# bxh1/VIDO-SLAM

Hardware: AMD Instinct MI355X
Metric: frames/sec end-to-end (flow+depth+track+local-BA) at 640x480; BA iters/sec (higher is better)
Workload: dtype f32

## Files before the change

### include/vido_c.h

```cpp
#ifndef VIDO_C_H
#define VIDO_C_H
#include <stdint.h>
#include <stddef.h>
#ifdef __cplusplus
extern "C" {
#endif

#define VIDO_OK              0
#define VIDO_E_INVALID      -1
#define VIDO_E_NO_DEVICE    -2
#define VIDO_E_HIP          -3
#define VIDO_E_CAPACITY     -4
#define VIDO_E_NOMEM        -5

#define VIDO_MAX_LEVELS 16

typedef struct vido_ctx vido_ctx;

typedef struct vido_keypoint { float x, y, size, angle, response; int32_t octave; } vido_keypoint;

typedef struct vido_config {
    int32_t device;
    int32_t width, height;
    int32_t max_batch;
// ... 115 lines not shown

typedef int (*vido_allreduce_fn)(void* user, void* dev_ptr, size_t count, int op);

int vido_ba_optimize(vido_ctx* ctx, vido_ba_problem* prob, vido_ba_result* result, vido_allreduce_fn allreduce, void* user);
int vido_rccl_unique_id(uint8_t id_out[128]);
int vido_rccl_init(vido_ctx* ctx, const uint8_t id[128], int rank, int world);
int vido_rccl_allreduce(void* user_ctx, void* dev_ptr, size_t count, int op);
int vido_rccl_destroy(vido_ctx* ctx);

typedef struct vido_ba_dynamic {
    int32_t n_H, n_dyn, n_tern, n_smooth;
    double* H_T;
    double* dyn_xyz;
    const int32_t* dyn_cam; const double* dyn_meas;
    const int32_t* tern_prev; const int32_t* tern_cur; const int32_t* tern_H;
    const int32_t* sm_i; const int32_t* sm_j;
    double info_dyn, info_tern, info_smooth, huber_dyn, huber_tern, huber_smooth;
} vido_ba_dynamic;
int vido_ba_optimize_dynamic(vido_ctx* ctx, vido_ba_problem* prob, vido_ba_dynamic* dyn, vido_ba_result* result,
                             vido_allreduce_fn allreduce, void* user);

int vido_correlation(vido_ctx* ctx, const float* first, const float* second, int B, int C, int H, int W, int stride,
                     float* out, int on_device);
int vido_det_order(vido_ctx* ctx, const float* scores, const long long* labels, const int* n_det, float confidence, int cap, long long* order, long long* labels_out, long long* n_live);
int vido_roi_levels(vido_ctx* ctx, const float* boxes, int n, float k_min, float k_max, int* out);
int vido_mask_logit_select(vido_ctx* ctx, const float* feat, const float* w, const float* b, const long long* labels, float* out, int n, int c, int hw, int classes);
int vido_bias_act(vido_ctx* ctx, float* x, const float* bias, int N, int C, int H, int W, float slope);
int vido_bias_unary(vido_ctx* ctx, float* x, const float* bias, int N, int C, int H, int W, int kind);
int vido_upcat_reflect(vido_ctx* ctx, const float* x, const float* skip, int C1, int C2, int h, int w, float* out);
int vido_minmax_norm_u16(vido_ctx* ctx, const float* d, const float* mm, int64_t n, int32_t* out);
int vido_bias_res_act(vido_ctx* ctx, float* x, const float* bias, const float* res, int N, int C, int H, int W, float slope);
int vido_area_feed(vido_ctx* ctx, const uint8_t* bgr, int H, int W, float* out, int OH, int OW, float div);
int vido_backwarp(vido_ctx* ctx, const float* x, const float* flow, int B, int C, int H, int W, float* out);
int vido_deconv4s2_depthwise(vido_ctx* ctx, const float* x, const float* weight, int B, int C, int H, int W, float input_slope, float* out);

int vido_conv1x1_supported(int cin, int cout, int hw);
int vido_conv1x1_layout(int cin, int cout, int hw);
int vido_conv1x1_set_arith(int arith);
int vido_conv1x1_range_flag(vido_ctx* ctx, int reset);
int vido_range_latch(vido_ctx* ctx, unsigned* dst);
int vido_conv1x1_bias_act(vido_ctx* ctx, const float* x, const float* w_packed, const float* bias, const float* residual, float* y, int cin, int cout, int hw, float slope);
int vido_deconv2x2_supported(int n, int cin, int cout, int h, int w);
int vido_deconv2x2_bias_act(vido_ctx* ctx, const float* x, const float* w_packed, const float* bias, float* y, int n, int cin, int cout, int h, int w, float slope);
int vido_conv1x1_bias_up2_act(vido_ctx* ctx, const float* x, const float* w_packed, const float* bias, const float* residual_half, float* y, int cin, int cout, int h, int w, float slope);

int vido_conv_kxk_c2(vido_ctx* ctx, const float* x, const float* w, const float* bias, const float* residual, float* y, int cin, int k, int h, int w_);
int vido_conv1x1_skinny(vido_ctx* ctx, const float* x, const float* w_packed, const float* bias, const float* residual, float* y, int cin, int cout, long long hw, float slope);

int vido_conv_direct_supported(int cin, int cout, int h, int w, int kh, int kw, int sh, int sw, int ph, int pw);
long long vido_conv_direct_packed_floats(int cin, int cout, int kh, int kw);
int vido_conv_direct_pack(const float* w, int cin, int cout, int kh, int kw, float* w_packed);
int vido_conv_direct_bias_act(vido_ctx* ctx, const float* x, const float* w_packed, const float* bias, float* y, int n, int cin, int cout, int h, int w,
                              int kh, int kw, int sh, int sw, int ph, int pw, float slope);

int vido_wino3x3_supported(int cin, int cout, int h, int w);
int vido_wino3x3_fills_chip(int n, int cout, int h, int w, int min_wgs);
long long vido_wino3x3_packed_floats(int cin, int cout);
int vido_wino3x3_pack(const float* w, int cin, int cout, float* u_packed);
int vido_wino3x3_bias_act(vido_ctx* ctx, const float* x, const float* u_packed, const float* bias, float* y, int n, int cin, int cout, int h, int w, float slope);
int vido_wino3x3_form(int n, int cin, int cout, int h, int w);
int vido_fc_h_splitk(int rows, int k, int outs);
int vido_fc_h(vido_ctx* ctx, const float* x, const void* w_packed, const float* bias, float* part, float* y, int rows, int k, int outs, float slope);
int vido_conv3x3_h_supported(int n, int cin, int cout, int h, int w);
int vido_conv3x3_h_workgroups(int n, int cout, int h, int w);
int vido_conv3x3_h_bias_act(vido_ctx* ctx, const float* x, const void* w_packed, const float* bias, float* y, int n, int cin, int cout, int h, int w, float slope);
long long vido_wino3x3_packed_floats_form(int cin, int cout, int form);
int vido_wino3x3_pack_form(const float* w, int cin, int cout, int form, float* u_packed);
int vido_wino3x3_bias_act_form(vido_ctx* ctx, const float* x, const float* u_packed, const float* bias, float* y, int n, int cin, int cout, int h, int w, float slope, int form);
int vido_gconv3x3_supported(int H, int W, int cpg_in, int cpg_out);
int64_t vido_gconv3x3_packed_size(int groups, int cpg_in, int cpg_out);
int vido_gconv3x3_bias_act(vido_ctx* ctx, const float* x, const float* in_bias, const float* w_packed, const float* bias, float* y, int groups, int cpg_in, int cpg_out, int H, int W, float slope);
int vido_gconv3x3_s2_supported(int H, int W, int cpg_in, int cpg_out);
int vido_gconv3x3_s2_bias_act(vido_ctx* ctx, const float* x, const float* w_packed, const float* bias, float* y, int groups, int cpg_in, int cpg_out, int H, int W, float slope);
int vido_lfn_reg_front(vido_ctx* ctx, const float* im1, const float* im2, const float* flow, const float* mean, float scale, int B, int C, int H, int W, float* out, int out_channels);
int vido_lfn_reg_tail(vido_ctx* ctx, const float* dist, const float* flow, const float* wx, const float* bx, const float* wy, const float* by, int B, int K, int H, int W, float* out);
int vido_roi_align(vido_ctx* ctx, const float* feat, int B, int C, int H, int W, const float* rois, int n_rois,
                   float spatial_scale, int pooled_h, int pooled_w, int sampling_ratio, float* out, int on_device);
int vido_nms(vido_ctx* ctx, const float* boxes_xyxy, const float* scores, int n, float thresh, int32_t* keep_out,
             int32_t* n_keep, int on_device);
int vido_nms_grouped(vido_ctx* ctx, const float* boxes_xyxy, const float* scores, const int32_t* groups, int n, float thresh,
                     int32_t* keep_out, int32_t* n_keep, int on_device);
int vido_nms_segments(vido_ctx* ctx, const float* boxes_xyxy, const int32_t* groups, const int32_t* seg_off, const int32_t* seg_n, int n_seg, int max_n, int total,
                      float thresh, int32_t* keep_out, int32_t* n_keep);
int vido_roi_align_fpn(vido_ctx* ctx, const float* const feat[4], const int H[4], const int W[4], const float scale[4], int C, const float* boxes, const int32_t* level,
                       int n, int pooled_h, int pooled_w, int sampling_ratio, float* out);
int vido_nchw_to_nhwc(vido_ctx* ctx, const float* src, int B, int C, int H, int W, float* dst);
int vido_roi_align_fpn_nhwc(vido_ctx* ctx, const float* const feat[4], const int H[4], const int W[4], const float scale[4], int C, const float* boxes, const int32_t* level,
                            int n, int pooled_h, int pooled_w, int sampling_ratio, float* out);
int vido_bawin_create(vido_ctx* ctx, int cap_frames, int cap_features);
int vido_bawin_push_frame(vido_ctx* ctx, int frame, int n, const double* meas, const float* xyz, const int32_t* asso);
int vido_bawin_set_labels(vido_ctx* ctx, int n, const int32_t* quads);
int vido_bawin_solve(vido_ctx* ctx, int start, int N, vido_ba_problem* prob, vido_ba_result* res, int32_t* n_obs_out, int32_t* n_pt_out);
int vido_bawin_read_points(vido_ctx* ctx, int frame, int n, float* xyz_out);
int vido_rpn_select(vido_ctx* ctx, int n_levels, const float* const* logits, const float* const* deltas, const int* h, const int* w, const int* stride, const float* cell_anchors,
                    int A, int K, int img_w, int img_h, float* boxes_out, float* scores_out, int32_t* n_out);
int vido_rpn_merge(vido_ctx* ctx, const float* boxes, const float* scores, const int32_t* keep, const int32_t* cnt, int n_levels, int K, int post_nms_top_n, int n_final,
                   float* out_boxes, float* out_scores, int32_t* n_valid);
int vido_det_class_sort(vido_ctx* ctx, const float* prob, const float* deltas, const float* proposals, const float* objectness, int N, int nc, float thresh, const float weights[4],
                        int img_w, int img_h, float* seg_boxes, int32_t* order, int32_t* seg_n);
int vido_det_select(vido_ctx* ctx, const float* prob, const float* seg_boxes, const int32_t* order, const int32_t* keep, const int32_t* cnt, int N, int nc, int detections_per_img, int cap,
                    int32_t* scratch, float* out_boxes, float* out_scores, int64_t* out_labels, int32_t* n_det);
int vido_mask_label_image(vido_ctx* ctx, const float* masks, const float* boxes, const int64_t* labels, int n, int M, int padding, float thresh, int H, int W, uint8_t* out);
int vido_box_decode(vido_ctx* ctx, const float* deltas, const float* boxes, int n, int k, const float weights[4],
                    float* out, int on_device);

int vido_pnp_ransac(vido_ctx* ctx, const float* pts3d, const float* pts2d, int n, double fx, double fy, double cx, double cy,
// ... 60 lines not shown
```

### vido-slam_amd/build.py

```python
import os, subprocess, glob, hashlib

HERE = os.path.dirname(os.path.abspath(__file__))
CSRC = os.path.join(HERE, "csrc")
LIB = os.path.join(HERE, "libvido_slam_hip.so")
import shlex as _shlex
FLAGS = _shlex.split(os.environ.get("VIDO_EXTRA_FLAGS", "")) + ["--offload-arch=gfx950", "-O3", "-std=c++17", "-fPIC", "-shared", "-ffp-contract=off",
         "-fno-fast-math", "-munsafe-fp-atomics", "-Wall", "-Wno-unused-function", "-Wno-unused-result", "-Wno-unused-value", "-pthread"]


def sources():
    return sorted(glob.glob(os.path.join(CSRC, "*.hip")) + glob.glob(os.path.join(CSRC, "*.cpp")))


def _stamp():
    h = hashlib.sha1()
    for p in sources() + sorted(glob.glob(os.path.join(CSRC, "*.hpp"))) + sorted(glob.glob(os.path.join(HERE, "..", "include", "*.h"))):
        h.update(open(p, "rb").read())
    h.update(" ".join(FLAGS).encode())
    return h.hexdigest()


def _obj_stamp(src):
    h = hashlib.sha1()
    h.update(open(src, "rb").read())
    for p in sorted(glob.glob(os.path.join(CSRC, "*.hpp"))) + sorted(glob.glob(os.path.join(HERE, "..", "include", "*.h"))) + sorted(glob.glob(os.path.join(HERE, "..", "include", "vido_slam", "*.h"))):
        h.update(open(p, "rb").read())
    h.update(" ".join(FLAGS + _file_flags(src)).encode())
    return h.hexdigest()


FILE_FLAGS = {"convdirect": ["-mllvm", "-amdgpu-mfma-vgpr-form"]}


_PROBED = {}


def _flag_ok(flags):
    key = " ".join(flags)
    if key not in _PROBED:
        import tempfile
        with tempfile.TemporaryDirectory() as d:
            src = os.path.join(d, "probe.hip"); open(src, "w").write("__global__ void k() {}\n")
            r = subprocess.run([os.environ.get("HIPCC", "/opt/rocm/bin/hipcc"), "--offload-arch=gfx950", "-c", "-x", "hip", src, "-o", os.path.join(d, "probe.o")] + flags,
                               stdout=subprocess.DEVNULL, stderr=subprocess.DEVNULL)
        _PROBED[key] = r.returncode == 0
    return _PROBED[key]


def _file_flags(src):
    stem = os.path.basename(src).split(".")[0]
    ff = FILE_FLAGS.get(stem, [])
    if ff and not _flag_ok(ff):
        ff = []
    return ff + _shlex.split(os.environ.get("VIDO_FLAGS_" + stem, ""))


def build(force=False, verbose=False, lib=None):
    lib = lib or LIB
    stamp_file = lib + ".stamp"
    stamp = _stamp() + "".join(" ".join(_file_flags(x)) for x in sources())
    if not force and os.path.exists(lib) and os.path.exists(stamp_file) and open(stamp_file).read() == stamp:
        return lib
    hipcc = os.environ.get("HIPCC", "/opt/rocm/bin/hipcc")
    objdir = os.path.join(HERE, "build")
    os.makedirs(objdir, exist_ok=True)
    cflags = [f for f in FLAGS if f != "-shared"]
    jobs, objs = [], []
    for s in sources():
        o = os.path.join(objdir, os.path.basename(s) + "." + _obj_stamp(s)[:16] + ".o")
        objs.append(o)
        if force or not os.path.exists(o):
            jobs.append([hipcc] + cflags + _file_flags(s) + ["-c", "-x", "hip", s, "-o", o])
    if jobs:
        from concurrent.futures import ThreadPoolExecutor
        def run(cmd):
            if verbose:
                print(" ".join(cmd))
            subprocess.check_call(cmd)
        with ThreadPoolExecutor(max_workers=min(len(jobs), os.cpu_count() or 4)) as ex:
            list(ex.map(run, jobs))
    subprocess.check_call([hipcc, "--offload-arch=gfx950", "-shared", "-fPIC", "-pthread", "-o", lib] + objs)
    live = set(objs)
    for o in glob.glob(os.path.join(objdir, "*.o")):
        if o not in live and lib == LIB:
# ... 20 lines not shown
```

### vido-slam_amd/nets/fuse.py

```python
import os
import torch
import torch.nn as nn
import torch.nn.functional as F


def _fold(conv, bn, eps):
    scale = bn.weight * (bn.running_var + eps).rsqrt()
    w = conv.weight * scale.reshape(-1, 1, 1, 1)
    b = bn.bias - bn.running_mean * scale
    if conv.bias is not None:
        b = b + conv.bias * scale
    return w.detach().contiguous(), b.detach().contiguous()


def _eps(bn):
    return float(getattr(bn, "eps", 0.0))


def fold_batchnorm(net, ops):
    from .maskrcnn import _Bottleneck, _Stem
    from .monodepth2 import _Basic, ResnetEncoder18, DepthDecoder
    n = 0
    for m in net.modules():
        if isinstance(m, _Bottleneck):
            m._w1, m._b1 = _fold(m.conv1, m.bn1, _eps(m.bn1)); m._w2, m._b2 = _fold(m.conv2, m.bn2, _eps(m.bn2)); m._w3, m._b3 = _fold(m.conv3, m.bn3, _eps(m.bn3)); n += 3
            if m.downsample is not None:
                m._wd, m._bd = _fold(m.downsample[0], m.downsample[1], _eps(m.downsample[1])); n += 1
            m._ep = ops.bias_res_act_
            c2 = m.conv2; m._w2p = None; m._ops = ops
            if c2.groups > 1 and tuple(c2.stride) == (1, 1) and tuple(c2.padding) == (1, 1) and tuple(c2.dilation) == (1, 1) and not os.environ.get("VIDO_NO_GCONV"):
                from .ops import pack_gconv3x3
                m._w2p = pack_gconv3x3(m._w2, c2.groups)
            elif (c2.groups > 1 and tuple(c2.stride) == (2, 2) and tuple(c2.padding) == (1, 1) and tuple(c2.dilation) == (1, 1) and ((c2.out_channels // c2.groups) % 32 == 0 or (c2.out_channels // c2.groups) in (8, 16))
                  and not os.environ.get("VIDO_NO_GCONV") and not os.environ.get("VIDO_NO_GCONV_S2")):
                from .ops import pack_gconv3x3
                m._w2p = pack_gconv3x3(m._w2, c2.groups)
            m._w1p = m._w3p = m._wdp = None; m._c1x1_min_tiles = 0
            mode = os.environ.get("VIDO_CONV1X1", "all")
            if not os.environ.get("VIDO_NO_CONV1X1") and hasattr(ops, "conv1x1_bias_act"):
                from .ops import PackedConv1x1
                m._w3p = PackedConv1x1.make(m._w3)
                if mode == "all":
                    if tuple(m.conv1.stride) == (1, 1): m._w1p = PackedConv1x1.make(m._w1)
                    if m.downsample is not None and tuple(m.downsample[0].stride) in ((1, 1), (2, 2)): m._wdp = PackedConv1x1.make(m._wd)
        elif isinstance(m, _Stem):
            m._w1, m._b1 = _fold(m.conv1, m.bn1, _eps(m.bn1)); m._ep = ops.bias_res_act_; n += 1
        elif isinstance(m, _Basic):
            m._w1, m._b1 = _fold(m.conv1, m.bn1, m.bn1.eps); m._w2, m._b2 = _fold(m.conv2, m.bn2, m.bn2.eps); n += 2
            if m.downsample is not None:
                m._wd, m._bd = _fold(m.downsample[0], m.downsample[1], m.downsample[1].eps); n += 1
            m._ep = ops.bias_res_act_
        elif isinstance(m, DepthDecoder):
            m._ops = ops if hasattr(ops, "upcat_reflect") and not os.environ.get("VIDO_NO_DEPTH_FUSED") else None
        elif isinstance(m, ResnetEncoder18):
            e = m.encoder
            w, b = _fold(e.conv1, e.bn1, e.bn1.eps)
            m._w1, m._b1 = w, b; m._ep = ops.bias_res_act_; n += 1
    return n


class Graphed:

    def __init__(self, fn, example_inputs, warmup=2):
        self.fn = fn
        self.static_in = [x.clone() for x in example_inputs]
        side = torch.cuda.Stream()
        side.wait_stream(torch.cuda.current_stream())
        with torch.cuda.stream(side):
            for _ in range(warmup):
                fn(*self.static_in)
        torch.cuda.current_stream().wait_stream(side)
        torch.cuda.synchronize()
        self.graph = torch.cuda.CUDAGraph()
        with torch.cuda.graph(self.graph):
            self.static_out = fn(*self.static_in)
        torch.cuda.synchronize()

    def __call__(self, *inputs):
        for d, s in zip(self.static_in, inputs):
            if d.data_ptr() != s.data_ptr():
                d.copy_(s, non_blocking=True)
        self.graph.replay()
        return self.static_out
```

### vido-slam_amd/nets/monodepth2.py

```python
import torch
import torch.nn as nn
import torch.nn.functional as F


class _Basic(nn.Module):
    def __init__(self, cin, cout, stride):
        super().__init__()
        self.conv1 = nn.Conv2d(cin, cout, 3, stride, 1, bias=False); self.bn1 = nn.BatchNorm2d(cout)
        self.conv2 = nn.Conv2d(cout, cout, 3, 1, 1, bias=False); self.bn2 = nn.BatchNorm2d(cout)
        self.downsample = None
        if stride != 1 or cin != cout:
            self.downsample = nn.Sequential(nn.Conv2d(cin, cout, 1, stride, bias=False), nn.BatchNorm2d(cout))

    _ep = None

    def forward(self, x):
        if self._ep is not None and x.is_cuda:
            ep = self._ep
            y = ep(F.conv2d(x, self._w1, None, self.conv1.stride, 1), self._b1, None, 0.0)
            sc = x if self.downsample is None else ep(F.conv2d(x, self._wd, None, self.downsample[0].stride), self._bd, None, 1.0)
            return ep(F.conv2d(y, self._w2, None, 1, 1), self._b2, sc.contiguous(), 0.0)
        y = F.relu(self.bn1(self.conv1(x)))
        y = self.bn2(self.conv2(y))
        return F.relu(y + (x if self.downsample is None else self.downsample(x)))


class _ResNet18Trunk(nn.Module):
    def __init__(self):
        super().__init__()
        self.conv1 = nn.Conv2d(3, 64, 7, 2, 3, bias=False); self.bn1 = nn.BatchNorm2d(64)
        self.layer1 = nn.Sequential(_Basic(64, 64, 1), _Basic(64, 64, 1))
        self.layer2 = nn.Sequential(_Basic(64, 128, 2), _Basic(128, 128, 1))
        self.layer3 = nn.Sequential(_Basic(128, 256, 2), _Basic(256, 256, 1))
        self.layer4 = nn.Sequential(_Basic(256, 512, 2), _Basic(512, 512, 1))
        self.fc = nn.Linear(512, 1000)


class ResnetEncoder18(nn.Module):
    num_ch_enc = (64, 64, 128, 256, 512)

    def __init__(self):
        super().__init__()
        self.encoder = _ResNet18Trunk()

    _ep = None

    def forward(self, image):
        e = self.encoder
        if self._ep is not None and image.is_cuda:
            x = self._ep(F.conv2d((image - 0.45) / 0.225, self._w1, None, 2, 3), self._b1, None, 0.0)
        else:
            x = F.relu(e.bn1(e.conv1((image - 0.45) / 0.225)))
        feats = [x]
        x = e.layer1(F.max_pool2d(x, 3, 2, 1)); feats.append(x)
        for layer in (e.layer2, e.layer3, e.layer4):
            x = layer(x); feats.append(x)
        return feats


class _Conv3x3(nn.Module):
    def __init__(self, cin, cout):
        super().__init__()
        self.pad = nn.ReflectionPad2d(1); self.conv = nn.Conv2d(int(cin), int(cout), 3)

    def forward(self, x):
        return self.conv(self.pad(x))


class _ConvBlock(nn.Module):
    def __init__(self, cin, cout):
        super().__init__()
        self.conv = _Conv3x3(cin, cout); self.nonlin = nn.ELU(inplace=True)

    def forward(self, x):
        return self.nonlin(self.conv(x))


class DepthDecoder(nn.Module):
    num_ch_dec = (16, 32, 64, 128, 256)

    def __init__(self, num_ch_enc=ResnetEncoder18.num_ch_enc, scales=range(4)):
        super().__init__()
        self.scales = list(scales); mods = []; self.index = {}
        for i in range(4, -1, -1):
            cin = num_ch_enc[-1] if i == 4 else self.num_ch_dec[i + 1]
            self.index[("upconv", i, 0)] = len(mods); mods.append(_ConvBlock(cin, self.num_ch_dec[i]))
            cin = self.num_ch_dec[i] + (num_ch_enc[i - 1] if i > 0 else 0)
            self.index[("upconv", i, 1)] = len(mods); mods.append(_ConvBlock(cin, self.num_ch_dec[i]))
        for s in self.scales:
            self.index[("dispconv", s)] = len(mods); mods.append(_Conv3x3(self.num_ch_dec[s], 1))
        self.decoder = nn.ModuleList(mods)

    _ops = None

    def forward_fused(self, feats):
        ops = self._ops; x = feats[-1]
        for i in range(4, -1, -1):
            b0 = self.decoder[self.index[("upconv", i, 0)]].conv; b1 = self.decoder[self.index[("upconv", i, 1)]].conv
            x = ops.bias_unary_(F.conv2d(b0.pad(x), b0.conv.weight, None), b0.conv.bias, "elu")
            x = ops.upcat_reflect(x, feats[i - 1].contiguous() if i > 0 else None)
            x = ops.bias_unary_(F.conv2d(x, b1.conv.weight, None), b1.conv.bias, "elu")
        d0 = self.decoder[self.index[("dispconv", 0)]]
        return {("disp", 0): ops.bias_unary_(F.conv2d(d0.pad(x), d0.conv.weight, None), d0.conv.bias, "sigmoid")}

    def forward(self, feats):
        if self._ops is not None and feats[-1].is_cuda and feats[-1].shape[0] == 1:
            return self.forward_fused(feats)
        out = {}; x = feats[-1]
        for i in range(4, -1, -1):
            x = self.decoder[self.index[("upconv", i, 0)]](x)
            x = F.interpolate(x, scale_factor=2, mode="nearest")
            if i > 0:
                x = torch.cat([x, feats[i - 1]], 1)
            x = self.decoder[self.index[("upconv", i, 1)]](x)
            if i in self.scales:
                out[("disp", i)] = torch.sigmoid(self.decoder[self.index[("dispconv", i)]](x))
        return out


class MonoDepth2(nn.Module):
    def __init__(self):
        super().__init__()
        self.encoder = ResnetEncoder18(); self.depth_decoder = DepthDecoder()

    @torch.no_grad()
    def forward(self, image):
        return self.depth_decoder(self.encoder(image))[("disp", 0)]


@torch.no_grad()
def analyse_depth(net, bgr, feed=(192, 640), ops=None):
    dev = next(net.parameters()).device
    if ops is not None and torch.is_tensor(bgr) and bgr.is_cuda and bgr.dtype == torch.uint8:
        H, W = bgr.shape[0], bgr.shape[1]
        x = ops.area_feed(bgr.contiguous(), feed, 255.0)
    else:
        t = (bgr.to(dev).flip(-1) if torch.is_tensor(bgr) else torch.as_tensor(bgr[:, :, ::-1].copy(), device=dev)).permute(2, 0, 1).float().unsqueeze(0)
        H, W = t.shape[2], t.shape[3]
        x = F.interpolate(t, size=feed, mode="area").div(255.0)
    disp = F.interpolate(net(x), size=(H, W), mode="bilinear", align_corners=False)[0, 0]
    if ops is not None and disp.is_cuda and hasattr(ops, "minmax_norm_u16"):
        return ops.minmax_norm_u16(disp)
    lo, hi = disp.min(), disp.max()
    return ((disp - lo) / (hi - lo + 1e-12) * 65536.0).clamp(0, 65535).to(torch.int32)
```

### vido-slam_amd/nets/ops.py

```python
import contextlib
import ctypes as C
import os
import torch

_WINO_MIN_WGS = int(os.environ.get("VIDO_WINO_MIN_WGS", "0"))
_CONV3X3_H_MIN_WGS = 0 if os.environ.get("VIDO_CONV3X3_H") == "0" else int(os.environ.get("VIDO_CONV3X3_H_MIN_WGS", "128"))
_CONVDIRECT_SET = os.environ.get("VIDO_CONVDIRECT_SET", "novalu")


def correlation_torch_reference(first, second, stride):
    a, b = first[:, :, ::stride, ::stride], second[:, :, ::stride, ::stride]
    pad = torch.nn.functional.pad(b, (3, 3, 3, 3))
    H, W = a.shape[2], a.shape[3]
    return torch.stack([(a * pad[:, :, p:p + H, o:o + W]).mean(1) for p in range(7) for o in range(7)], 1)


class HipOps:

    _range_safe = 0

    def __init__(self, ctx):
        self.ctx = ctx

    @property
# ... 302 lines not shown
        out = torch.empty((N, cout, H, W), device=x.device, dtype=torch.float32)
        self.gconv_flops = getattr(self, "gconv_flops", 0.0) + 2.0 * N * cout * cin * 9 * H * W
        self._adopt_stream()
        self.ctx._check(self.ctx.lib.vido_conv3x3_h_bias_act(self.ctx.h, C.c_void_p(x.data_ptr()), C.c_void_p(w_packed.data_ptr()), C.c_void_p(bias.data_ptr()) if bias is not None else None,
                                                             C.c_void_p(out.data_ptr()), int(N), int(cin), int(cout), int(H), int(W), C.c_float(slope)))
        return out

    def fc_h(self, x, w_packed, bias, outs, slope=1.0):
        assert x.is_cuda and x.is_contiguous() and x.dtype == torch.float32 and x.dim() == 2
        rows, k = int(x.shape[0]), int(x.shape[1])
        S = int(self.ctx.lib.vido_fc_h_splitk(rows, k, int(outs)))
        if S <= 0:
            return None
        assert w_packed.dtype == torch.int16 and w_packed.numel() == 2 * outs * (k + 1), "fc_h: weight not packed (pack_conv1x1(w[:, :, None, None], 3))"
        part = torch.empty((S, rows, outs), device=x.device, dtype=torch.float32); y = torch.empty((rows, outs), device=x.device, dtype=torch.float32)
        self.gconv_flops = getattr(self, "gconv_flops", 0.0) + 2.0 * rows * k * outs
        self._adopt_stream()
        self.ctx._check(self.ctx.lib.vido_fc_h(self.ctx.h, C.c_void_p(x.data_ptr()), C.c_void_p(w_packed.data_ptr()), C.c_void_p(bias.data_ptr()) if bias is not None else None,
                                               C.c_void_p(part.data_ptr()), C.c_void_p(y.data_ptr()), rows, k, int(outs), C.c_float(slope)))
        return y

    def fc_h_linear(self, lin, x, slope=1.0):
        w = lin.weight
        if not x.is_cuda or x.dtype != torch.float32 or x.dim() != 2 or os.environ.get("VIDO_NO_FC_H") or self._range_safe or int(self.ctx.lib.vido_fc_h_splitk(int(x.shape[0]), int(w.shape[1]), int(w.shape[0]))) <= 0:
            return None
        key = (w.data_ptr(), w._version, str(x.device))
        if getattr(lin, "_fch_key", None) != key:
            lin._fch_w = pack_conv1x1(w.detach().reshape(int(w.shape[0]), int(w.shape[1]), 1, 1), 3).to(x.device); lin._fch_key = key
        return self.fc_h(x.contiguous(), lin._fch_w, lin.bias, int(w.shape[0]), slope)

    def conv_direct_conv(self, conv, x, slope):
        w = conv.weight
        kh, kw = int(w.shape[2]), int(w.shape[3]); sh, sw = (int(v) for v in conv.stride); ph, pw = (int(v) for v in conv.padding)
        if _CONVDIRECT_SET == "novalu" and (kh, kw) in ((3, 3), (7, 7)) and int(w.shape[0]) >= 32:
            return None
        if (tuple(conv.dilation) != (1, 1) or conv.groups != 1 or getattr(conv, "padding_mode", "zeros") != "zeros" or not x.is_cuda or x.dtype != torch.float32
                or not self.ctx.lib.vido_conv_direct_supported(int(w.shape[1]), int(w.shape[0]), int(x.shape[2]), int(x.shape[3]), kh, kw, sh, sw, ph, pw)
                or 4 * x.numel() >= 1 << 30):
            return None
        N, cin, H, W = x.shape; cout = int(w.shape[0])
        Ho, Wo = (H + 2 * ph - kh) // sh + 1, (W + 2 * pw - kw) // sw + 1
        if 4 * N * cout * Ho * Wo >= 1 << 30:
            return None
        key = (w.data_ptr(), w._version, str(x.device))
        if getattr(conv, "_cd_key", None) != key:
            conv._cd_w = pack_conv_direct(w).to(x.device); conv._cd_key = key
        x = x.contiguous()
        out = torch.empty((N, cout, Ho, Wo), device=x.device, dtype=torch.float32)
        self.gconv_flops = getattr(self, "gconv_flops", 0.0) + 2.0 * N * cout * cin * kh * kw * Ho * Wo
        self._adopt_stream()
        b = conv.bias
        self.ctx._check(self.ctx.lib.vido_conv_direct_bias_act(self.ctx.h, C.c_void_p(x.data_ptr()), C.c_void_p(conv._cd_w.data_ptr()), C.c_void_p(b.data_ptr()) if b is not None else None,
                                                               C.c_void_p(out.data_ptr()), int(N), int(cin), cout, int(H), int(W), kh, kw, sh, sw, ph, pw, C.c_float(slope)))
        return out

    def lfn_reg_front(self, im1, im2, flow, scale, feat):
        im1 = im1.contiguous(); im2 = im2.contiguous(); flow = flow.contiguous()
        B, Cc, H, W = im1.shape
        out = torch.empty((B, 3 + feat.shape[1], H, W), device=im1.device, dtype=torch.float32)
        mean = flow.flatten(2).mean(2).contiguous()
        self._adopt_stream()
        self.ctx._check(self.ctx.lib.vido_lfn_reg_front(self.ctx.h, C.c_void_p(im1.data_ptr()), C.c_void_p(im2.data_ptr()), C.c_void_p(flow.data_ptr()), C.c_void_p(mean.data_ptr()),
                                                        C.c_float(scale), B, Cc, H, W, C.c_void_p(out.data_ptr()), out.shape[1]))
        out[:, 3:] = feat
        return out

    def lfn_reg_tail(self, dist, flow, scale_x, scale_y, k):
        dist = dist.contiguous(); flow = flow.contiguous()
        B, nd, H, W = dist.shape
        assert nd == k * k
        out = torch.empty((B, 2, H, W), device=dist.device, dtype=torch.float32)
        self._adopt_stream()
        self.ctx._check(self.ctx.lib.vido_lfn_reg_tail(self.ctx.h, C.c_void_p(dist.data_ptr()), C.c_void_p(flow.data_ptr()), C.c_void_p(scale_x.weight.data_ptr()), C.c_void_p(scale_x.bias.data_ptr()),
                                                       C.c_void_p(scale_y.weight.data_ptr()), C.c_void_p(scale_y.bias.data_ptr()), B, int(k), H, W, C.c_void_p(out.data_ptr())))
        return out

    def roi_align(self, feat, rois, output_size, spatial_scale, sampling_ratio):
        if not feat.is_cuda:
            raise RuntimeError("HipOps.roi_align needs CUDA(HIP) tensors; there is no CPU fallback")
        feat = feat.contiguous().float(); rois = rois.contiguous().float()
        B, Cc, H, W = feat.shape; ph, pw = output_size
        out = torch.empty((rois.shape[0], Cc, ph, pw), device=feat.device, dtype=torch.float32)
        self._adopt_stream()
        self.ctx._check(self.ctx.lib.vido_roi_align(self.ctx.h, C.c_void_p(feat.data_ptr()), B, Cc, H, W, C.c_void_p(rois.data_ptr()), rois.shape[0],
                                                    C.c_float(spatial_scale), ph, pw, sampling_ratio, C.c_void_p(out.data_ptr()), 1))
        return out

    def box_decode(self, deltas, boxes, weights):
        deltas = deltas.contiguous().float(); boxes = boxes.contiguous().float(); n = deltas.shape[0]
        out = torch.empty_like(deltas)
        if n:
            w = (C.c_float * 4)(*[float(x) for x in weights])
            self._adopt_stream()
            self.ctx._check(self.ctx.lib.vido_box_decode(self.ctx.h, C.c_void_p(deltas.data_ptr()), C.c_void_p(boxes.data_ptr()), n, deltas.shape[1] // 4, w,
                                                         C.c_void_p(out.data_ptr()), 1))
        return out

    def nms_grouped(self, boxes, scores, groups, thresh):
        if not boxes.is_cuda:
            raise RuntimeError("HipOps.nms_grouped needs CUDA(HIP) tensors; there is no CPU fallback")
        if boxes.shape[0] == 0:
            return torch.zeros((0,), dtype=torch.int64, device=boxes.device)
        order = torch.sort(scores, descending=True, stable=True)[1]
        n = boxes.shape[0]
        if n <= 65536:
            order = order[torch.sort(groups[order], stable=True)[1]]
# ... 317 lines not shown
```

Measured before the change: 127.6.

## Add native MFMA conv kernel path for monodepth2 encoder and decoder

Adds a dedicated fp32 MFMA convolution kernel for the depth network. It fuses input normalisation, reflect padding, nearest upsample plus skip concatenation, bias, residual add and ReLU/ELU/sigmoid into a single launch, with split-K reduction through shared memory, plus a native maxpool. The ResNet18 encoder blocks, the stem and the depth decoder route through it by default, replacing F.conv2d followed by separate epilogue, pad, upsample and concat ops. The aim is to cut launch count and intermediate memory traffic. The cost is a large new kernel whose Kahan-style compensated summation and plain fp32 MFMA may be slower than the vendor convolution library for some shapes.

```diff
diff --git a/include/vido_c.h b/include/vido_c.h
--- a/include/vido_c.h
+++ b/include/vido_c.h
@@ -191,6 +191,12 @@
 int vido_conv_direct_pack(const float* w, int cin, int cout, int kh, int kw, float* w_packed);
 int vido_conv_direct_bias_act(vido_ctx* ctx, const float* x, const float* w_packed, const float* bias, float* y, int n, int cin, int cout, int h, int w,
                               int kh, int kw, int sh, int sw, int ph, int pw, float slope);
+
+int vido_conv_depth_supported(int mode, int n, int cin, int c1, int cout, int h, int w, int k, int stride, int pad);
+int vido_conv_depth_form(int n, int cin, int cout, int ho, int wo, int k);
+int vido_conv_depth(vido_ctx* ctx, int mode, const float* x, const float* skip, int c1, const float* w_packed, const float* bias, const float* res, float* y,
+                    int n, int cin, int cout, int h, int w, int k, int stride, int pad, int act);
+int vido_maxpool3x3s2(vido_ctx* ctx, const float* x, float* y, int n, int c, int h, int w);
 
 int vido_wino3x3_supported(int cin, int cout, int h, int w);
 int vido_wino3x3_fills_chip(int n, int cout, int h, int w, int min_wgs);
diff --git a/vido-slam_amd/build.py b/vido-slam_amd/build.py
--- a/vido-slam_amd/build.py
+++ b/vido-slam_amd/build.py
@@ -29,7 +29,7 @@
     return h.hexdigest()
 
 
-FILE_FLAGS = {"convdirect": ["-mllvm", "-amdgpu-mfma-vgpr-form"]}
+FILE_FLAGS = {"convdirect": ["-mllvm", "-amdgpu-mfma-vgpr-form"], "convdepth": ["-mllvm", "-amdgpu-mfma-vgpr-form"]}
 
 
 _PROBED = {}
diff --git a/vido-slam_amd/csrc/convdepth.hip b/vido-slam_amd/csrc/convdepth.hip
--- /dev/null
+++ b/vido-slam_amd/csrc/convdepth.hip
@@ -0,0 +1,271 @@
+#include "common.hpp"
+
+namespace {
+typedef float f32x16 __attribute__((ext_vector_type(16)));
+#define DP_OOB 0x40000000u
+
+struct DpArgs {
+    const float* x; const float* skip; const float* wp; const float* bias; const float* res; float* y;
+    int N, Cin, C1, Cout, H, W, Ho, Wo, S, P, npix, cgroups, total, cpr, cpp;
+    unsigned xbytes, sbytes, wbytes;
+};
+
+constexpr int dp_unroll(int kh, int kw) { return kh * kw >= 25 ? 2 : 4; }
+
+__device__ __forceinline__ int dp_reflect(int i, int n) { return i < 0 ? -i : (i >= n ? 2 * n - 2 - i : i); }
+
+template <int K, int MODE, int ACT, int CBW, int KS>
+__global__ __launch_bounds__(512) void k_conv_depth(DpArgs A)
+{
+    constexpr int T = K * K, U = dp_unroll(K, K), WPG = KS > 4 ? KS : 4;
+    const int lane = threadIdx.x & 63, w = __builtin_amdgcn_readfirstlane(threadIdx.x >> 6);
+    const int per = gridDim.x >> 3, wg = (blockIdx.x & 7) * per + (blockIdx.x >> 3);
+    const int item = wg * (WPG / KS) + w / KS, ks = w % KS;
+    const bool live = item < A.total;
+    const int itc = live ? item : A.total - 1;
+    const int tile = itc / A.cgroups, cg = itc - tile * A.cgroups;
+    const int n = lane & 31, kk = lane >> 5;
+    const int g = tile * 32 + n, gc = min(g, A.npix - 1), hwo = A.Ho * A.Wo, hw = A.H * A.W;
+    const bool pv = g < A.npix;
+    const int img = gc / hwo, rem = gc - img * hwo, oy = rem / A.Wo, ox = rem - oy * A.Wo;
+    const int iy0 = oy * A.S - A.P, ix0 = ox * A.S - A.P;
+    const int hx = A.H >> 1, wx = A.W >> 1;
+    const unsigned odd_oob = ((A.Cin & 1) && kk) ? DP_OOB : 0u;
+    const __amdgpu_buffer_rsrc_t xr = __builtin_amdgcn_make_buffer_rsrc((void*)A.x, 0, A.xbytes, 0x00020000);
+    const __amdgpu_buffer_rsrc_t sr = __builtin_amdgcn_make_buffer_rsrc((void*)(MODE == 3 && A.skip ? A.skip : A.x), 0, MODE == 3 && A.skip ? A.sbytes : 0u, 0x00020000);
+    const __amdgpu_buffer_rsrc_t wr = __builtin_amdgcn_make_buffer_rsrc((void*)A.wp, 0, A.wbytes, 0x00020000);
+    const unsigned wl = 4u * (unsigned)lane;
+    const int cpr = A.cpr, cpp = A.cpp, nmain = ((A.Cin >> 1) / U) * U, spt = cpp / U;
+    const int c1p = A.C1 >> 1;
+    const unsigned cstep = MODE == 3 ? 8u * (unsigned)(hx * wx) : 8u * (unsigned)hw, sstep = 8u * (unsigned)hw;
+    const unsigned wblk = 4u * 64u * (unsigned)(T * cpp);
+    const int S = T * spt, s0 = live ? ks * S / KS : 0, s1 = live ? (ks + 1) * S / KS : 0, nst = s1 - s0;
+    auto tap_off = [&](int t, unsigned& vt, unsigned& vs) {
+        const int ky = t / K, kx = t - ky * K;
+        int iy = iy0 + ky, ix = ix0 + kx;
+        if (MODE >= 2) {
+            iy = dp_reflect(iy, A.H); ix = dp_reflect(ix, A.W);
+            if (MODE == 3) {
+                vt = pv ? 4u * (unsigned)((img * A.C1 + kk) * hx * wx + (iy >> 1) * wx + (ix >> 1)) : DP_OOB;
+                vs = pv ? 4u * (unsigned)((img * (A.Cin - A.C1) + kk) * hw + iy * A.W + ix) : DP_OOB;
+            } else {
+                vt = pv ? 4u * (unsigned)((img * A.Cin + kk) * hw + iy * A.W + ix) : DP_OOB;
+                vs = vt;
+            }
+        } else {
+            const bool tv = pv && (unsigned)iy < (unsigned)A.H && (unsigned)ix < (unsigned)A.W;
+            vt = tv ? 4u * (unsigned)((img * A.Cin + kk) * hw + iy * A.W + ix) : DP_OOB;
+            vs = vt;
+        }
+    };
+    int lt = s0 / spt, lcp = (s0 - lt * spt) * U;
+    unsigned wsc = 4u * 64u * (unsigned)(cg * CBW * T * cpp + lt * cpp + lcp);
+    unsigned vt, vs;
+    tap_off(lt, vt, vs);
+    auto load_step = [&](float (&b)[U], float (&a)[CBW][U]) {
+        if (MODE == 3 && lcp >= c1p) {
+#pragma unroll
+            for (int u = 0; u < U; u++)
+                b[u] = __builtin_bit_cast(float, __builtin_amdgcn_raw_buffer_load_b32(sr, vs, (unsigned)(lcp - c1p + u) * sstep, 0));
+        } else if (lcp < nmain) {
+#pragma unroll
+            for (int u = 0; u < U; u++) {
+                float v = __builtin_bit_cast(float, __builtin_amdgcn_raw_buffer_load_b32(xr, vt, (unsigned)(lcp + u) * cstep, 0));
+                if (MODE == 1) v = (vt & DP_OOB) ? 0.f : (v - 0.45f) / 0.225f;
+                b[u] = v;
+            }
+        } else {
+#pragma unroll
+            for (int u = 0; u < U; u++) {
+                const int c = lcp + u;
+                const unsigned vo = c >= cpr ? DP_OOB : (c == cpr - 1 ? (vt | odd_oob) : vt);
+                float v = __builtin_bit_cast(float, __builtin_amdgcn_raw_buffer_load_b32(xr, vo, cstep * (unsigned)min(c, cpr - 1), 0));
+                if (MODE == 1) v = (vo & DP_OOB) ? 0.f : (v - 0.45f) / 0.225f;
+                b[u] = v;
+            }
+        }
+#pragma unroll
+        for (int u = 0; u < U; u++)
+#pragma unroll
+            for (int i = 0; i < CBW; i++)
+                a[i][u] = __builtin_bit_cast(float, __builtin_amdgcn_raw_buffer_load_b32(wr, wl, wsc + (unsigned)i * wblk + 256u * (unsigned)u, 0));
+        lcp += U; wsc += 256u * (unsigned)U;
+        if (lcp >= cpp) { lcp = 0; lt++; tap_off(min(lt, T - 1), vt, vs); }
+    };
+    f32x16 blk[CBW], sum[CBW], cmp[CBW];
+#pragma unroll
+    for (int i = 0; i < CBW; i++)
+#pragma unroll
+        for (int q = 0; q < 16; q++) { sum[i][q] = 0.f; cmp[i][q] = 0.f; }
+    float bq[4][U], aq[4][CBW][U];
+#pragma unroll
+    for (int j = 0; j < 3; j++)
+        if (j < nst) load_step(bq[j], aq[j]);
+    for (int st = 0; st < nst; st += 4) {
+#pragma unroll
+        for (int i = 0; i < CBW; i++)
+#pragma unroll
+            for (int q = 0; q < 16; q++) blk[i][q] = 0.f;
+#pragma unroll
+        for (int j = 0; j < 4; j++) {
+            if (st + j < nst) {
+                if (st + j + 3 < nst) load_step(bq[(j + 3) & 3], aq[(j + 3) & 3]);
+#pragma unroll
+                for (int u = 0; u < U; u++)
+#pragma unroll
+                    for (int i = 0; i < CBW; i++) blk[i] = __builtin_amdgcn_mfma_f32_32x32x2f32(aq[j][i][u], bq[j][u], blk[i], 0, 0, 0);
+            }
+        }
+#pragma unroll
+        for (int i = 0; i < CBW; i++) {
+            const f32x16 yv = blk[i] - cmp[i], t = sum[i] + yv;
+            cmp[i] = (t - sum[i]) - yv; sum[i] = t;
+        }
+    }
+    f32x16 acc0[CBW];
+#pragma unroll
+    for (int i = 0; i < CBW; i++) acc0[i] = sum[i] - cmp[i];
+    const size_t ob = (size_t)img * A.Cout * hwo + rem;
+    auto epilogue = [&](int i, int q, float v) {
+        const int co = (cg * CBW + i) * 32 + 8 * (q >> 2) + 4 * kk + (q & 3);
+        if (!live || !pv || co >= A.Cout) return;
+        v = v + A.bias[co];
+        if (A.res) v = v + A.res[ob + (size_t)co * hwo];
+        if (ACT == 1) v = fmaxf(v, 0.f);
+        else if (ACT == 2) v = v > 0.f ? v : expf(v) - 1.f;
+        else if (ACT == 3) v = 1.f / (1.f + expf(-v));
+        A.y[ob + (size_t)co * hwo] = v;
+    };
+    if (KS == 1) {
+#pragma unroll
+        for (int i = 0; i < CBW; i++)
+#pragma unroll
+            for (int q = 0; q < 16; q++) epilogue(i, q, acc0[i][q]);
+        return;
+    }
+    __shared__ float red[KS > 1 ? WPG * CBW * 16 * 64 : 1];
+#pragma unroll
+    for (int i = 0; i < CBW; i++)
+#pragma unroll
+        for (int q = 0; q < 16; q++) red[((w * CBW + i) * 16 + q) * 64 + lane] = acc0[i][q];
+    __syncthreads();
+    const int w0 = w - ks;
+#pragma unroll
+    for (int r = 0; r < CBW * 16; r++) {
+        if (r % KS != ks) continue;
+        float v = red[(w0 * CBW * 16 + r) * 64 + lane];
+#pragma unroll
+        for (int s = 1; s < KS; s++) v += red[((w0 + s) * CBW * 16 + r) * 64 + lane];
+        epilogue(r / 16, r % 16, v);
+    }
+}
+
+inline int dp_cpp(int cin, int k) { const int u = dp_unroll(k, k), cpr = (cin + 1) / 2; return ((cpr + u - 1) / u) * u; }
+
+inline void dp_form(int n, int cin, int cout, int ho, int wo, int k, int& ks, int& cbw)
+{
+    const long long ntile = ((long long)n * ho * wo + 31) / 32, cb = (cout + 31) / 32;
+    const int steps = k * k * (dp_cpp(cin, k) / dp_unroll(k, k));
+    cbw = (cb >= 2 && ntile * ((cb + 1) / 2) >= 2048) ? 2 : 1;
+    const long long items = ntile * ((cb + cbw - 1) / cbw);
+    ks = 1;
+    while (ks < 8 && items * ks < 2048 && steps / (2 * ks) >= 4) ks *= 2;
+    if (ks > 4) cbw = 1;
+}
+}
+
+extern "C" {
+
+int vido_conv_depth_supported(int mode, int n, int cin, int c1, int cout, int h, int w, int k, int stride, int pad)
+{
+    if (mode < 0 || mode > 3 || n < 1 || cin < 1 || cout < 1 || h < 1 || w < 1 || !(k == 1 || k == 3 || k == 7) || stride < 1 || stride > 2 || pad < 0 || pad >= k) return 0;
+    if (mode >= 2 && (k != 3 || stride != 1 || pad != 1 || h < 2 || w < 2 || (cin & 7))) return 0;
+    if (mode == 3 && ((h & 1) || (w & 1) || c1 < 8 || (c1 & 7) || c1 > cin)) return 0;
+    if (mode != 3 && c1 != 0) return 0;
+    const long long ho = (h + 2 * pad - k) / stride + 1, wo = (w + 2 * pad - k) / stride + 1;
+    if (h + 2 * pad < k || w + 2 * pad < k || ho < 1 || wo < 1) return 0;
+    return 4ll * n * cin * h * w < (1ll << 30) && 4ll * n * cout * ho * wo < (1ll << 30) && (long long)n * ho * wo < (1ll << 28);
+}
+
+int vido_conv_depth_form(int n, int cin, int cout, int ho, int wo, int k)
+{
+    int ks, cbw;
+    dp_form(n, cin, cout, ho, wo, k, ks, cbw);
+    return ks;
+}
+
+int vido_conv_depth(vido_ctx* ctx, int mode, const float* x, const float* skip, int c1, const float* w_packed, const float* bias, const float* res, float* y,
+                    int n, int cin, int cout, int h, int w, int k, int stride, int pad, int act)
+{
+    if (!ctx) return VIDO_E_INVALID;
+    if (!x || !w_packed || !bias || !y || x == y || (skip && skip == y) || (res && res == y) || act < 0 || act > 3 || !vido_conv_depth_supported(mode, n, cin, c1, cout, h, w, k, stride, pad)
+        || (mode == 3 && c1 < cin && !skip) || (((uintptr_t)x | (uintptr_t)y | (uintptr_t)w_packed | (uintptr_t)skip | (uintptr_t)res) & 3))
+        return vido_set_error(ctx, VIDO_E_INVALID, "conv_depth: no kernel for mode %d, %d -> %d channels, %d x %d taps, stride %d on %d x %d x %d", mode, cin, cout, k, k, stride, n, h, w);
+    const int ho = (h + 2 * pad - k) / stride + 1, wo = (w + 2 * pad - k) / stride + 1;
+    HIP_TRY(ctx, hipSetDevice(ctx->device));
+    hipStream_t st = ctx->has_ext_stream ? ctx->ext_stream : ctx->stream;
+    int ks, cbw;
+    dp_form(n, cin, cout, ho, wo, k, ks, cbw);
+    const long long npix = (long long)n * ho * wo, ntile = (npix + 31) / 32, cgroups = ((cout + 31) / 32 + cbw - 1) / cbw, total = ntile * cgroups;
+    const long long xfl = mode == 3 ? (long long)n * c1 * (h / 2) * (w / 2) : (long long)n * cin * h * w;
+    DpArgs A{x, skip, w_packed, bias, res, y, n, cin, mode == 3 ? c1 : cin, cout, h, w, ho, wo, stride, pad, (int)npix, (int)cgroups, (int)total, (cin + 1) / 2, dp_cpp(cin, k),
+             (unsigned)(4 * xfl), (unsigned)(4ll * n * (cin - c1) * h * w), (unsigned)(4ll * vido_conv_direct_packed_floats(cin, cout, k, k))};
+    const int wpg = ks > 4 ? ks : 4, ipg = wpg / ks;
+    const long long nwg = (total + ipg - 1) / ipg;
+    const dim3 grid((unsigned)(8 * ((nwg + 7) / 8))), blk(64 * wpg);
+#define DP_KS(K_, M_, A_, C_) do { switch (ks) { \
+        case 1: hipLaunchKernelGGL((k_conv_depth<K_, M_, A_, C_, 1>), grid, blk, 0, st, A); break; \
+        case 2: hipLaunchKernelGGL((k_conv_depth<K_, M_, A_, C_, 2>), grid, blk, 0, st, A); break; \
+        case 4: hipLaunchKernelGGL((k_conv_depth<K_, M_, A_, C_, 4>), grid, blk, 0, st, A); break; \
+        default: hipLaunchKernelGGL((k_conv_depth<K_, M_, A_, C_, 8>), grid, blk, 0, st, A); } } while (0)
+#define DP_CBW(K_, M_, A_) do { if (cbw == 2 && ks <= 4) DP_KS(K_, M_, A_, 2); else DP_KS(K_, M_, A_, 1); } while (0)
+    if (k == 7 && mode == 1 && act == 1) DP_CBW(7, 1, 1);
+    else if (k == 3 && mode == 0 && act == 1) DP_CBW(3, 0, 1);
+    else if (k == 1 && mode == 0 && act == 0) DP_CBW(1, 0, 0);
+    else if (k == 3 && mode == 2 && act == 2) DP_CBW(3, 2, 2);
+    else if (k == 3 && mode == 3 && act == 2) DP_CBW(3, 3, 2);
+    else if (k == 3 && mode == 2 && act == 3) DP_CBW(3, 2, 3);
+    else if (k == 3 && mode == 0 && act == 0) DP_CBW(3, 0, 0);
+    else if (k == 3 && mode == 2 && act == 0) DP_CBW(3, 2, 0);
+    else return vido_set_error(ctx, VIDO_E_INVALID, "conv_depth: no instance for %d x %d taps, mode %d, activation %d", k, k, mode, act);
+#undef DP_CBW
+#undef DP_KS
+    HIP_TRY(ctx, hipGetLastError());
+    return VIDO_OK;
+}
+
+}
+
+namespace {
+__global__ __launch_bounds__(256) void k_maxpool3s2(const float* __restrict__ x, float* __restrict__ y, int H, int W, int Ho, int Wo, long long total)
+{
+    const long long i = blockIdx.x * (long long)blockDim.x + threadIdx.x;
+    if (i >= total) return;
+    const int ox = (int)(i % Wo), oy = (int)((i / Wo) % Ho);
+    const long long c = i / ((long long)Wo * Ho);
+    const float* xc = x + c * H * W;
+    float m = -INFINITY;
+    for (int dy = -1; dy <= 1; dy++) {
+        const int iy = 2 * oy + dy;
+        if ((unsigned)iy >= (unsigned)H) continue;
+        for (int dx = -1; dx <= 1; dx++) {
+            const int ix = 2 * ox + dx;
+            if ((unsigned)ix < (unsigned)W) { const float v = xc[iy * W + ix]; m = (v > m || v != v) ? v : m; }
+        }
+    }
+    y[i] = m;
+}
+}
+
+extern "C" int vido_maxpool3x3s2(vido_ctx* ctx, const float* x, float* y, int n, int c, int h, int w)
+{
+    if (!ctx) return VIDO_E_INVALID;
+    if (!x || !y || x == y || n < 1 || c < 1 || h < 1 || w < 1 || (long long)n * c * h * w >= (1ll << 40)) return vido_set_error(ctx, VIDO_E_INVALID, "maxpool3x3s2: bad arguments");
+    HIP_TRY(ctx, hipSetDevice(ctx->device));
+    hipStream_t st = ctx->has_ext_stream ? ctx->ext_stream : ctx->stream;
+    const int ho = (h - 1) / 2 + 1, wo = (w - 1) / 2 + 1;
+    const long long total = (long long)n * c * ho * wo;
+    hipLaunchKernelGGL(k_maxpool3s2, dim3((unsigned)((total + 255) / 256)), dim3(256), 0, st, x, y, h, w, ho, wo, total);
+    HIP_TRY(ctx, hipGetLastError());
+    return VIDO_OK;
+}
diff --git a/vido-slam_amd/nets/fuse.py b/vido-slam_amd/nets/fuse.py
--- a/vido-slam_amd/nets/fuse.py
+++ b/vido-slam_amd/nets/fuse.py
@@ -19,7 +19,8 @@
 
 def fold_batchnorm(net, ops):
     from .maskrcnn import _Bottleneck, _Stem
-    from .monodepth2 import _Basic, ResnetEncoder18, DepthDecoder
+    from .monodepth2 import _Basic, _Conv3x3, ResnetEncoder18, DepthDecoder
+    from .ops import pack_conv_direct
     n = 0
     for m in net.modules():
         if isinstance(m, _Bottleneck):
@@ -50,13 +51,28 @@
             if m.downsample is not None:
                 m._wd, m._bd = _fold(m.downsample[0], m.downsample[1], m.downsample[1].eps); n += 1
             m._ep = ops.bias_res_act_
+            m._nat = ops if _depth_native(ops) else None
+            if m._nat is not None:
+                dev = m._w1.device
+                m._w1p = pack_conv_direct(m._w1).to(dev); m._w2p = pack_conv_direct(m._w2).to(dev)
+                m._wdp = pack_conv_direct(m._wd).to(dev) if m.downsample is not None else None
         elif isinstance(m, DepthDecoder):
             m._ops = ops if hasattr(ops, "upcat_reflect") and not os.environ.get("VIDO_NO_DEPTH_FUSED") else None
+            m._nat = ops if _depth_native(ops) else None
+            if m._nat is not None:
+                convs = [c.conv.conv if isinstance(c.conv, _Conv3x3) else c.conv for c in m.decoder]
+                m._wp = [pack_conv_direct(c.weight).to(c.weight.device) for c in convs]
         elif isinstance(m, ResnetEncoder18):
             e = m.encoder
             w, b = _fold(e.conv1, e.bn1, e.bn1.eps)
             m._w1, m._b1 = w, b; m._ep = ops.bias_res_act_; n += 1
+            m._nat = ops if _depth_native(ops) else None
+            m._w1p = pack_conv_direct(w).to(w.device) if m._nat is not None else None
     return n
+
+
+def _depth_native(ops):
+    return hasattr(ops, "conv_depth") and not os.environ.get("VIDO_NO_DEPTH_NATIVE") and not os.environ.get("VIDO_NO_DEPTH_FUSED")
 
 
 class Graphed:
diff --git a/vido-slam_amd/nets/monodepth2.py b/vido-slam_amd/nets/monodepth2.py
--- a/vido-slam_amd/nets/monodepth2.py
+++ b/vido-slam_amd/nets/monodepth2.py
@@ -13,8 +13,14 @@
             self.downsample = nn.Sequential(nn.Conv2d(cin, cout, 1, stride, bias=False), nn.BatchNorm2d(cout))
 
     _ep = None
+    _nat = None
 
     def forward(self, x):
+        if self._nat is not None and x.is_cuda:
+            ops = self._nat; x = x.contiguous(); s = int(self.conv1.stride[0]); cout = int(self._w1.shape[0])
+            y = ops.conv_depth(x, self._w1p, self._b1, cout, 3, s, 1, "zero", "relu")
+            sc = x if self.downsample is None else ops.conv_depth(x, self._wdp, self._bd, cout, 1, int(self.downsample[0].stride[0]), 0, "zero", None)
+            return ops.conv_depth(y, self._w2p, self._b2, cout, 3, 1, 1, "zero", "relu", res=sc)
         if self._ep is not None and x.is_cuda:
             ep = self._ep
             y = ep(F.conv2d(x, self._w1, None, self.conv1.stride, 1), self._b1, None, 0.0)
@@ -44,9 +50,17 @@
         self.encoder = _ResNet18Trunk()
 
     _ep = None
+    _nat = None
 
     def forward(self, image):
         e = self.encoder
+        if self._nat is not None and image.is_cuda:
+            x = self._nat.conv_depth(image.contiguous(), self._w1p, self._b1, 64, 7, 2, 3, "norm", "relu")
+            feats = [x]
+            x = e.layer1(self._nat.maxpool3x3s2(x)); feats.append(x)
+            for layer in (e.layer2, e.layer3, e.layer4):
+                x = layer(x); feats.append(x)
+            return feats
         if self._ep is not None and image.is_cuda:
             x = self._ep(F.conv2d((image - 0.45) / 0.225, self._w1, None, 2, 3), self._b1, None, 0.0)
         else:
@@ -92,6 +106,17 @@
         self.decoder = nn.ModuleList(mods)
 
     _ops = None
+    _nat = None
+
+    def forward_native(self, feats):
+        ops = self._nat; x = feats[-1].contiguous()
+        def conv(key, x, mode, act, skip=None):
+            j = self.index[key]; c = self.decoder[j]; c = c.conv if isinstance(c, _ConvBlock) else c
+            return ops.conv_depth(x, self._wp[j], c.conv.bias, int(c.conv.out_channels), 3, 1, 1, mode, act, skip=skip)
+        for i in range(4, -1, -1):
+            x = conv(("upconv", i, 0), x, "reflect", "elu")
+            x = conv(("upconv", i, 1), x, "upcat", "elu", feats[i - 1].contiguous() if i > 0 else None)
+        return {("disp", 0): conv(("dispconv", 0), x, "reflect", "sigmoid")}
 
     def forward_fused(self, feats):
         ops = self._ops; x = feats[-1]
@@ -104,6 +129,8 @@
         return {("disp", 0): ops.bias_unary_(F.conv2d(d0.pad(x), d0.conv.weight, None), d0.conv.bias, "sigmoid")}
 
     def forward(self, feats):
+        if self._nat is not None and feats[-1].is_cuda:
+            return self.forward_native(feats)
         if self._ops is not None and feats[-1].is_cuda and feats[-1].shape[0] == 1:
             return self.forward_fused(feats)
         out = {}; x = feats[-1]
diff --git a/vido-slam_amd/nets/ops.py b/vido-slam_amd/nets/ops.py
--- a/vido-slam_amd/nets/ops.py
+++ b/vido-slam_amd/nets/ops.py
@@ -378,6 +378,41 @@
         b = conv.bias
         self.ctx._check(self.ctx.lib.vido_conv_direct_bias_act(self.ctx.h, C.c_void_p(x.data_ptr()), C.c_void_p(conv._cd_w.data_ptr()), C.c_void_p(b.data_ptr()) if b is not None else None,
                                                                C.c_void_p(out.data_ptr()), int(N), int(cin), cout, int(H), int(W), kh, kw, sh, sw, ph, pw, C.c_float(slope)))
+        return out
+
+    _DEPTH_MODES = {"zero": 0, "norm": 1, "reflect": 2, "upcat": 3}
+    _DEPTH_ACTS = {None: 0, "relu": 1, "elu": 2, "sigmoid": 3}
+
+    def conv_depth(self, x, w_packed, bias, cout, k, stride=1, pad=1, mode="zero", act=None, res=None, skip=None):
+        assert x.is_cuda and x.is_contiguous() and x.dtype == torch.float32 and w_packed.is_cuda and bias is not None
+        m = self._DEPTH_MODES[mode]
+        N, c1, h, w = (int(v) for v in x.shape)
+        if m == 3:
+            h, w = 2 * h, 2 * w
+            if skip is not None:
+                assert skip.is_contiguous() and skip.dtype == torch.float32 and skip.shape[0] == N and tuple(skip.shape[2:]) == (h, w)
+            cin = c1 + (int(skip.shape[1]) if skip is not None else 0)
+        else:
+            cin, c1 = c1, 0
+        if not self.ctx.lib.vido_conv_depth_supported(m, N, cin, c1, int(cout), h, w, int(k), int(stride), int(pad)):
+            raise RuntimeError("conv_depth: no kernel for mode %s, %d -> %d channels, %dx%d stride %d on %d x %d" % (mode, cin, cout, k, k, stride, h, w))
+        Ho, Wo = (h + 2 * pad - k) // stride + 1, (w + 2 * pad - k) // stride + 1
+        out = torch.empty((N, int(cout), Ho, Wo), device=x.device, dtype=torch.float32)
+        if res is not None:
+            assert res.shape == out.shape and res.is_contiguous() and res.dtype == torch.float32
+        self.gconv_flops = getattr(self, "gconv_flops", 0.0) + 2.0 * N * cout * cin * k * k * Ho * Wo
+        self._adopt_stream()
+        self.ctx._check(self.ctx.lib.vido_conv_depth(self.ctx.h, m, C.c_void_p(x.data_ptr()), C.c_void_p(skip.data_ptr()) if skip is not None else None, c1,
+                                                     C.c_void_p(w_packed.data_ptr()), C.c_void_p(bias.data_ptr()), C.c_void_p(res.data_ptr()) if res is not None else None,
+                                                     C.c_void_p(out.data_ptr()), N, cin, int(cout), h, w, int(k), int(stride), int(pad), self._DEPTH_ACTS[act]))
+        return out
+
+    def maxpool3x3s2(self, x):
+        assert x.is_cuda and x.is_contiguous() and x.dtype == torch.float32
+        N, Cc, H, W = (int(v) for v in x.shape)
+        out = torch.empty((N, Cc, (H - 1) // 2 + 1, (W - 1) // 2 + 1), device=x.device, dtype=torch.float32)
+        self._adopt_stream()
+        self.ctx._check(self.ctx.lib.vido_maxpool3x3s2(self.ctx.h, C.c_void_p(x.data_ptr()), C.c_void_p(out.data_ptr()), N, Cc, H, W))
         return out
 
     def lfn_reg_front(self, im1, im2, flow, scale, feat):
```

Result: no change. 128.6, median of 6 (+0.8%).
